# XiSHEN0220/RANSAC-Flow

Hardware: AMD Instinct MI355X
Metric: aligned image-pairs/sec @480×640, 1/2/4/8 MI355X; max-abs flow Δ vs ref (higher is better)
Workload: dtype f32

## Files before the change

### ransac-flow_amd/csrc/conv3x3s.hip

```cpp
#include "common.h"
#include "conv_epilogue.h"
#include "group.h"
#include <stdlib.h>

namespace {

typedef __bf16 bf16x8 __attribute__((ext_vector_type(8)));
typedef __bf16 bf16x2 __attribute__((ext_vector_type(2)));
typedef float f32x2 __attribute__((ext_vector_type(2)));
typedef unsigned u32x4 __attribute__((ext_vector_type(4)));

constexpr int PT_C = 16, PC = PT_C + 2;
template <int WM> struct Geo {
    static constexpr int BM = 64 * WM, WN = 4 / WM, PT_R = 4 * WN, PR = PT_R + 2, PP = PR * PC;
    static constexpr int B_ITEMS = 2 * PP, NBI = (B_ITEMS + 255) / 256;
};

struct C3SArgs {
    const float* in; const u32x4* wS; const float* scale; const float* shift; const float* res; float* out;
    int N, Cin, H, W, Cout, act, Mpad;
    int tilesM, tilesW, tilesS;
};

__device__ __forceinline__ unsigned pack_bf16(float a, float b) {
    const f32x2 v = {a, b};
    const bf16x2 h = __builtin_convertvector(v, bf16x2);
    unsigned u;
    __builtin_memcpy(&u, &h, 4);
    return u;
}
__device__ __forceinline__ void split_pair(float a, float b, unsigned& hi, unsigned& mid, unsigned& lo) {
    hi = pack_bf16(a, b);
    const float ra = a - __uint_as_float(hi << 16), rb = b - __uint_as_float(hi & 0xffff0000u);
    mid = pack_bf16(ra, rb);
    lo = pack_bf16(ra - __uint_as_float(mid << 16), rb - __uint_as_float(mid & 0xffff0000u));
}
__device__ __forceinline__ bf16x8 as_frag(const u32x4& w) {
    bf16x8 f;
    __builtin_memcpy(&f, &w, 16);
    return f;
}

typedef const __attribute__((address_space(1))) void* gptr_t;
typedef __attribute__((address_space(3))) void* lptr_t;

template <int OFF>
__device__ __forceinline__ void lds_rd(u32x4& d, unsigned addr) {
    asm volatile("ds_read_b128 %0, %1 offset:%2" : "=v"(d) : "v"(addr), "n"(OFF));
}
__device__ __forceinline__ void lds_wait8(u32x4& a, u32x4& b, u32x4& c, u32x4& d, u32x4& e, u32x4& f, u32x4& g, u32x4& h) {
    asm volatile("s_waitcnt lgkmcnt(0)" : "+v"(a), "+v"(b), "+v"(c), "+v"(d), "+v"(e), "+v"(f), "+v"(g), "+v"(h));
}
__device__ __forceinline__ void lds_wait4(u32x4& a, u32x4& b, u32x4& c, u32x4& d) {
    asm volatile("s_waitcnt lgkmcnt(0)" : "+v"(a), "+v"(b), "+v"(c), "+v"(d));
}

template <int WM, bool ADMA>
__device__ __forceinline__ void conv3x3_split_body(const C3SArgs& a, const unsigned bx) {
    using G = Geo<WM>;
    constexpr int TM = 2;
    constexpr int BM = G::BM, PT_R = G::PT_R, PP = G::PP, B_ITEMS = G::B_ITEMS, NBI = G::NBI;
    constexpr int A_WORDS = 3 * 2 * BM;
    constexpr int NA = (A_WORDS + 255) / 256;
    __shared__ u32x4 As[2][3][2][BM];
    __shared__ u32x4 Bs[2][3][2][PP];
    __shared__ float s_scale[BM], s_shift[BM];

    const int t = threadIdx.x, lane = t & 63, wave = __builtin_amdgcn_readfirstlane(t >> 6);
    const int wm = WM == 2 ? wave >> 1 : 0, wn = WM == 2 ? wave & 1 : wave;
    const int lrow = lane >> 5, lcol = lane & 31;
    const size_t HW = (size_t)a.H * a.W;
    const int nwg = a.tilesM * a.tilesW * a.tilesS;
    const int nk = a.Cin / 16;
    const int Hs = a.H + 1;

    int m0, row0, col0;
    {
        const int v = (int)bx, q = nwg / 8, r = nwg % 8, xcd = v % 8, j = v / 8;
        int bid = (xcd < r ? xcd * (q + 1) : r * (q + 1) + (xcd - r) * q) + j;
        m0 = (bid % a.tilesM) * BM; bid /= a.tilesM;
        col0 = (bid % a.tilesW) * PT_C;
        row0 = (bid / a.tilesW) * PT_R;
    }
    constexpr int A_ROWS = 256 / BM;
    const u32x4* wsrc = a.wS + (size_t)(t / BM) * a.Mpad + m0 + t % BM;
    auto a_on = [&](int j) { return (j + 1) * 256 <= A_WORDS || t + 256 * j < A_WORDS; };
    const float* bsrc[NBI];
    bool b_ok[NBI], b_on[NBI];
    int b_word[NBI];
#pragma unroll
    for (int u = 0; u < NBI; ++u) {
        const int it = t + 256 * u;
        b_on[u] = it < B_ITEMS;
        const int h = (b_on[u] ? it : 0) / PP, pp = (b_on[u] ? it : 0) % PP;
        const int pr = pp / PC, pc = pp % PC;
        const int sr = row0 - 1 + pr, x = col0 - 1 + pc;
        const int n = sr >= 0 ? sr / Hs : 0, y = sr >= 0 ? sr - n * Hs : 0;
        b_ok[u] = b_on[u] && sr >= 0 && n < a.N && y < a.H && x >= 0 && x < a.W;
        bsrc[u] = b_ok[u] ? a.in + ((size_t)n * a.Cin + 8 * h) * HW + (size_t)y * a.W + x : a.in;
        b_word[u] = h * PP + pp;
    }
    u32x4 ra[NA];
    float rb[8];
    auto load_a = [&](int q) {
#pragma unroll
        for (int j = 0; j < NA; ++j)
            ra[j] = wsrc[((size_t)q * 6 + (a_on(j) ? A_ROWS * j : 0)) * a.Mpad];
    };
    auto store_a = [&](int buf) {
#pragma unroll
        for (int j = 0; j < NA; ++j)
            if (a_on(j)) (&As[buf][0][0][0])[t + 256 * j] = ra[j];
    };
    auto dma_a = [&](int q, int buf) {
#pragma unroll
        for (int j = 0; j < NA; ++j)
            if ((j + 1) * 256 <= A_WORDS || wave < (A_WORDS - 256 * j) / 64)
                __builtin_amdgcn_global_load_lds((gptr_t)(wsrc + ((size_t)q * 6 + A_ROWS * j) * a.Mpad),
                                                 (lptr_t)(&As[buf][0][0][0] + 256 * j + 64 * wave), 16, 0, 0);
    };
    auto load_b = [&](int kb, int u) {
#pragma unroll
        for (int i = 0; i < 8; ++i) rb[i] = bsrc[u][((size_t)kb * 16 + i) * HW];
    };
    auto store_b = [&](int buf, int u) {
        if (!b_on[u]) return;
        u32x4 hi, mid, lo;
#pragma unroll
        for (int i = 0; i < 4; ++i) {
            unsigned h_, m_, l_;
            split_pair(b_ok[u] ? rb[2 * i] : 0.0f, b_ok[u] ? rb[2 * i + 1] : 0.0f, h_, m_, l_);
            hi[i] = h_; mid[i] = m_; lo[i] = l_;
        }
        u32x4* dst = &Bs[buf][0][0][0] + b_word[u];
        dst[0] = hi;
        dst[2 * PP] = mid;
        dst[4 * PP] = lo;
    };
    if (t < BM) {
        const int m = m0 + t;
        s_scale[t] = (a.scale && m < a.Cout) ? a.scale[m] : 1.0f;
        s_shift[t] = (a.shift && m < a.Cout) ? a.shift[m] : 0.0f;
    }
    if (ADMA) dma_a(0, 0);
    else { load_a(0); store_a(0); }
#pragma unroll
    for (int u = 0; u < NBI; ++u) { load_b(0, u); store_b(0, u); }
    if (ADMA) asm volatile("s_waitcnt vmcnt(0)" ::: "memory");
    else load_a(1);
    if (nk > 1) load_b(1, 0);
    __syncthreads();

    f32x16 acc[TM][2], low[TM][2];
#pragma unroll
    for (int i = 0; i < TM; ++i)
#pragma unroll
        for (int j = 0; j < 2; ++j)
#pragma unroll
            for (int r = 0; r < 16; ++r) { acc[i][j][r] = 0.0f; low[i][j][r] = 0.0f; }

    const int a_base = lrow * BM + wm * TM * 32 + lcol;
    int b_base[2];
#pragma unroll
    for (int j = 0; j < 2; ++j) b_base[j] = lrow * PP + (4 * wn + 2 * j + (lcol >> 4)) * PC + (lcol & 15);
    const int nq = 9 * nk;
    const unsigned as_lds = (unsigned)(uintptr_t)(lptr_t)&As[0][0][0][0], bs_lds = (unsigned)(uintptr_t)(lptr_t)&Bs[0][0][0][0];

    for (int kb = 0; kb < nk; ++kb) {
        const u32x4* bimg = &Bs[kb & 1][0][0][0];
#pragma unroll
        for (int tap = 0; tap < 9; ++tap) {
            const int q = kb * 9 + tap;
            const u32x4* aimg = &As[q & 1][0][0][0];
            const int toff = (tap / 3) * PC + tap % 3;
            bf16x8 a0[TM], a1[TM], b0[2], b1[2];
            u32x4 ra0[2], ra1[2], rb0[2], rb1[2];
            unsigned a_addr = 0, b_addr[2] = {0, 0};
            if constexpr (ADMA) {
                static_assert(TM == 2, "hand-written fragment reads: two channel tiles per wavefront");
                a_addr = as_lds + (unsigned)(((q & 1) * A_WORDS + a_base) * 16);
                b_addr[0] = bs_lds + (unsigned)(((kb & 1) * 6 * PP + b_base[0] + toff) * 16);
                b_addr[1] = bs_lds + (unsigned)(((kb & 1) * 6 * PP + b_base[1] + toff) * 16);
                lds_rd<0>(ra0[0], a_addr); lds_rd<512>(ra0[1], a_addr);
                lds_rd<2 * BM * 16>(ra1[0], a_addr); lds_rd<2 * BM * 16 + 512>(ra1[1], a_addr);
                lds_rd<0>(rb0[0], b_addr[0]); lds_rd<0>(rb0[1], b_addr[1]);
                lds_rd<2 * PP * 16>(rb1[0], b_addr[0]); lds_rd<2 * PP * 16>(rb1[1], b_addr[1]);
            } else {
#pragma unroll
                for (int i = 0; i < TM; ++i) {
                    a0[i] = as_frag(aimg[a_base + i * 32]);
                    a1[i] = as_frag(aimg[2 * BM + a_base + i * 32]);
                }
#pragma unroll
                for (int j = 0; j < 2; ++j) {
                    b0[j] = as_frag(bimg[b_base[j] + toff]);
                    b1[j] = as_frag(bimg[2 * PP + b_base[j] + toff]);
                }
            }
            if (!ADMA) {
                if (q + 1 < nq) store_a((q + 1) & 1);
                if (q + 2 < nq) load_a(q + 2);
            }
            int b_next = -1, b_kb = 0;
            if (kb + 1 < nk) {
                if (NBI == 2) {
                    if (tap == 3) { store_b((kb + 1) & 1, 0); b_next = 1; b_kb = kb + 1; }
                    if (tap == 7) store_b((kb + 1) & 1, 1);
                } else {
                    if (tap == 2) { store_b((kb + 1) & 1, 0); b_next = 1; b_kb = kb + 1; }
                    if (tap == 5) { store_b((kb + 1) & 1, 1); b_next = NBI - 1; b_kb = kb + 1; }
                    if (tap == 8) store_b((kb + 1) & 1, NBI - 1);
                }
            }
            if (tap == 8 && kb + 2 < nk) { b_next = 0; b_kb = kb + 2; }
            const bool b_req = b_next >= 0;
            if (ADMA && q + 1 < nq) dma_a(q + 1, (q + 1) & 1);
            if (!ADMA && b_req) { if (b_next == 0) load_b(b_kb, 0); else if (b_next == 1) load_b(b_kb, 1); else load_b(b_kb, NBI - 1); }
            __builtin_amdgcn_sched_barrier(0);
            if constexpr (ADMA) {
                lds_wait8(ra0[0], ra0[1], ra1[0], ra1[1], rb0[0], rb0[1], rb1[0], rb1[1]);
#pragma unroll
                for (int i = 0; i < 2; ++i) { a0[i] = as_frag(ra0[i]); a1[i] = as_frag(ra1[i]); b0[i] = as_frag(rb0[i]); b1[i] = as_frag(rb1[i]); }
            }
#pragma unroll
            for (int i = 0; i < TM; ++i)
#pragma unroll
                for (int j = 0; j < 2; ++j) {
                    low[i][j] = __builtin_amdgcn_mfma_f32_32x32x16_bf16(a1[i], b1[j], low[i][j], 0, 0, 0);
                    low[i][j] = __builtin_amdgcn_mfma_f32_32x32x16_bf16(a1[i], b0[j], low[i][j], 0, 0, 0);
                }
#pragma unroll
            for (int i = 0; i < TM; ++i)
#pragma unroll
                for (int j = 0; j < 2; ++j) low[i][j] = __builtin_amdgcn_mfma_f32_32x32x16_bf16(a0[i], b1[j], low[i][j], 0, 0, 0);
            __builtin_amdgcn_sched_barrier(0);
            if constexpr (ADMA) {
                lds_rd<4 * BM * 16>(ra1[0], a_addr); lds_rd<4 * BM * 16 + 512>(ra1[1], a_addr);
                lds_rd<4 * PP * 16>(rb1[0], b_addr[0]); lds_rd<4 * PP * 16>(rb1[1], b_addr[1]);
            } else {
#pragma unroll
                for (int i = 0; i < TM; ++i) a1[i] = as_frag(aimg[4 * BM + a_base + i * 32]);
#pragma unroll
                for (int j = 0; j < 2; ++j) b1[j] = as_frag(bimg[4 * PP + b_base[j] + toff]);
            }
            if (ADMA && b_req) {
                __builtin_amdgcn_sched_barrier(0);
                if (b_next == 0) load_b(b_kb, 0); else if (b_next == 1) load_b(b_kb, 1); else load_b(b_kb, NBI - 1);
                __builtin_amdgcn_sched_barrier(0);
            }
#pragma unroll
            for (int i = 0; i < TM; ++i)
#pragma unroll
                for (int j = 0; j < 2; ++j) acc[i][j] = __builtin_amdgcn_mfma_f32_32x32x16_bf16(a0[i], b0[j], acc[i][j], 0, 0, 0);
            __builtin_amdgcn_sched_barrier(0);
            if constexpr (ADMA) {
                lds_wait4(ra1[0], ra1[1], rb1[0], rb1[1]);
#pragma unroll
                for (int i = 0; i < 2; ++i) { a1[i] = as_frag(ra1[i]); b1[i] = as_frag(rb1[i]); }
            }
#pragma unroll
            for (int i = 0; i < TM; ++i)
#pragma unroll
                for (int j = 0; j < 2; ++j) {
                    low[i][j] = __builtin_amdgcn_mfma_f32_32x32x16_bf16(a1[i], b0[j], low[i][j], 0, 0, 0);
                    low[i][j] = __builtin_amdgcn_mfma_f32_32x32x16_bf16(a0[i], b1[j], low[i][j], 0, 0, 0);
                }
            __builtin_amdgcn_sched_barrier(0);
            if (ADMA) {
                asm volatile("s_waitcnt vmcnt(0) lgkmcnt(0)" ::: "memory");
                __builtin_amdgcn_s_barrier();
            } else {
                __syncthreads();
            }
        }
    }
#pragma unroll
    for (int i = 0; i < TM; ++i)
#pragma unroll
        for (int j = 0; j < 2; ++j)
#pragma unroll
            for (int r = 0; r < 16; ++r) acc[i][j][r] += low[i][j][r];

    size_t pix_off[2];
    bool pix_ok[2];
#pragma unroll
    for (int j = 0; j < 2; ++j) {
        const int sr = row0 + 4 * wn + 2 * j + (lcol >> 4), x = col0 + (lcol & 15);
        const int n = sr / Hs, y = sr - n * Hs;
        pix_ok[j] = n < a.N && y < a.H && x < a.W;
        pix_off[j] = pix_ok[j] ? (size_t)n * a.Cout * HW + (size_t)y * a.W + x : 0;
    }
    conv_epilogue<TM, 2, false>(acc, s_scale, s_shift, a.res, a.out, a.act, a.Cout, HW, m0, wm, lrow, pix_off, pix_ok, m0 + BM <= a.Cout);
}

template <int TM, bool ADMA>
__global__ __launch_bounds__(256, 2) void conv3x3_split_kernel(C3SArgs a) {
    conv3x3_split_body<TM, ADMA>(a, blockIdx.x);
}

template <int TM, bool ADMA>
__global__ __launch_bounds__(256, 2) void conv3x3_split_group_kernel(RfxGroupArgs<C3SArgs> g) {
    const unsigned y = blockIdx.y;
    if (blockIdx.x >= g.gx[y]) return;
    conv3x3_split_body<TM, ADMA>(g.p[y], blockIdx.x);
}

template <int TM, bool ADMA>
static int c3s_group_launch(const void* blob, const unsigned* gx, int n, hipStream_t st) {
    return rfx_group_launch_impl<C3SArgs>(conv3x3_split_group_kernel<TM, ADMA>, 256, blob, gx, n, st);
}

template <int TM, bool ADMA>
int launch_split3_a(C3SArgs& a, hipStream_t st) {
    a.tilesM = (a.Cout + 64 * TM - 1) / (64 * TM);
    a.tilesW = (a.W + PT_C - 1) / PT_C;
    const long long rows = (long long)a.N * (a.H + 1) - 1;
    a.tilesS = (int)((rows + Geo<TM>::PT_R - 1) / Geo<TM>::PT_R);
    const long long nwg = (long long)a.tilesM * a.tilesW * a.tilesS;
    if (nwg > 0x7fffffffLL) return RFX_E_LIMIT;
    if (rfx_group_recording()) return rfx_group_record(&c3s_group_launch<TM, ADMA>, &a, sizeof(a), (unsigned)nwg);
    hipLaunchKernelGGL((conv3x3_split_kernel<TM, ADMA>), dim3((unsigned)nwg), dim3(256), 0, st, a);
    RFX_LAUNCH_CHECK();
    return RFX_OK;
}

template <int TM>
int launch_split3(C3SArgs& a, hipStream_t st) {
    static const bool adma = !(getenv("RFX_C3S_ADMA") && atoi(getenv("RFX_C3S_ADMA")) == 0);
    return adma ? launch_split3_a<TM, true>(a, st) : launch_split3_a<TM, false>(a, st);
}

constexpr int S2_PR = 2 * 8 + 1, S2_PC = 33, S2_PP = S2_PR * S2_PC;
constexpr int S2_ITEMS = 2 * S2_PP, S2_NBI = (S2_ITEMS + 255) / 256;

struct C3S2Args {
    const float* in; const u32x4* wS; const float* scale; const float* shift; const float* res; float* out;
    int N, Cin, H, W, Ho, Wo, Cout, act, Mpad;
    int tilesM, tilesW, tilesS;
};

__device__ __forceinline__ void conv3x3_split_s2_body(const C3S2Args& a, const unsigned bx) {
    constexpr int TM = 2, BM = 128;
    constexpr int NA = 3;
    __shared__ u32x4 As[2][3][2][BM];
    __shared__ u32x4 Bs[3][2][S2_PP];
    __shared__ float s_scale[BM], s_shift[BM];

    const int t = threadIdx.x, lane = t & 63, wave = __builtin_amdgcn_readfirstlane(t >> 6);
    const int wm = wave >> 1, wn = wave & 1;
    const int lrow = lane >> 5, lcol = lane & 31;
    const size_t HW = (size_t)a.H * a.W, HWo = (size_t)a.Ho * a.Wo;
    const int nwg = a.tilesM * a.tilesW * a.tilesS;
    const int nk = a.Cin / 16;
    const int Hs = a.Ho + 1, Hin = 2 * Hs;

    int m0, row0, col0;
    {
        const int v = (int)bx, q = nwg / 8, r = nwg % 8, xcd = v % 8, j = v / 8;
        int bid = (xcd < r ? xcd * (q + 1) : r * (q + 1) + (xcd - r) * q) + j;
        m0 = (bid % a.tilesM) * BM; bid /= a.tilesM;
        col0 = (bid % a.tilesW) * 16;
        row0 = (bid / a.tilesW) * 8;
    }
    const u32x4* wsrc = a.wS + (size_t)(t / BM) * a.Mpad + m0 + t % BM;
    const float* bsrc[S2_NBI];
    bool b_ok[S2_NBI];
    int b_word[S2_NBI];
#pragma unroll
    for (int u = 0; u < S2_NBI; ++u) {
        const int it = t + 256 * u;
        const bool on = it < S2_ITEMS;
        const int h = (on ? it : 0) / S2_PP, pp = (on ? it : 0) % S2_PP;
        const int pr = pp / S2_PC, pc = pp % S2_PC;
        const int si = 2 * row0 - 1 + pr, x = 2 * col0 - 1 + pc;
        const int n = si >= 0 ? si / Hin : 0, y = si >= 0 ? si - n * Hin : 0;
        b_ok[u] = on && si >= 0 && n < a.N && y < a.H && x >= 0 && x < a.W;
        bsrc[u] = b_ok[u] ? a.in + ((size_t)n * a.Cin + 8 * h) * HW + (size_t)y * a.W + x : a.in;
        b_word[u] = on ? h * S2_PP + pr * S2_PC + (pc & 1) * 17 + (pc >> 1) : -1;
    }
    auto dma_a = [&](int q, int buf) {
#pragma unroll
        for (int j = 0; j < NA; ++j)
            __builtin_amdgcn_global_load_lds((gptr_t)(wsrc + ((size_t)q * 6 + 2 * j) * a.Mpad), (lptr_t)(&As[buf][0][0][0] + 256 * j + 64 * wave),
                                             16, 0, 0);
    };
    auto stage_b = [&](int kb) {
        float rb[4][8];
#pragma unroll
        for (int u = 0; u < 4; ++u)
#pragma unroll
            for (int i = 0; i < 8; ++i) rb[u][i] = bsrc[u][((size_t)kb * 16 + i) * HW];
        auto put = [&](const float (&v)[8], int u) {
            if (b_word[u] < 0) return;
            u32x4 hi, mid, lo;
#pragma unroll
            for (int i = 0; i < 4; ++i) {
                unsigned h_, m_, l_;
                split_pair(b_ok[u] ? v[2 * i] : 0.0f, b_ok[u] ? v[2 * i + 1] : 0.0f, h_, m_, l_);
                hi[i] = h_; mid[i] = m_; lo[i] = l_;
            }
            u32x4* dst = &Bs[0][0][0] + b_word[u];
            dst[0] = hi;
            dst[2 * S2_PP] = mid;
            dst[4 * S2_PP] = lo;
        };
#pragma unroll
        for (int u = 0; u < 4; ++u) put(rb[u], u);
        float r4[8];
#pragma unroll
        for (int i = 0; i < 8; ++i) r4[i] = bsrc[4][((size_t)kb * 16 + i) * HW];
        put(r4, 4);
    };
    if (t < BM) {
        const int m = m0 + t;
        s_scale[t] = (a.scale && m < a.Cout) ? a.scale[m] : 1.0f;
        s_shift[t] = (a.shift && m < a.Cout) ? a.shift[m] : 0.0f;
    }
    dma_a(0, 0);

    f32x16 acc[TM][2], low[TM][2];
#pragma unroll
    for (int i = 0; i < TM; ++i)
#pragma unroll
        for (int j = 0; j < 2; ++j)
#pragma unroll
            for (int r = 0; r < 16; ++r) { acc[i][j][r] = 0.0f; low[i][j][r] = 0.0f; }

    const int a_base = lrow * BM + wm * TM * 32 + lcol;
    int b_base[2];
#pragma unroll
    for (int j = 0; j < 2; ++j) b_base[j] = lrow * S2_PP + 2 * (4 * wn + 2 * j + (lcol >> 4)) * S2_PC + (lcol & 15);
    const int nq = 9 * nk;
    const u32x4* bimg = &Bs[0][0][0];

    for (int kb = 0; kb < nk; ++kb) {
        stage_b(kb);
        asm volatile("s_waitcnt vmcnt(0)" ::: "memory");
        __syncthreads();
#pragma unroll
        for (int tap = 0; tap < 9; ++tap) {
            const int q = kb * 9 + tap;
            const u32x4* aimg = &As[q & 1][0][0][0];
            const int toff = (tap / 3) * S2_PC + (tap % 3 & 1) * 17 + (tap % 3 >> 1);
            bf16x8 a0[TM], a1[TM], b0[2], b1[2];
#pragma unroll
            for (int i = 0; i < TM; ++i) {
                a0[i] = as_frag(aimg[a_base + i * 32]);
                a1[i] = as_frag(aimg[2 * BM + a_base + i * 32]);
            }
#pragma unroll
            for (int j = 0; j < 2; ++j) {
                b0[j] = as_frag(bimg[b_base[j] + toff]);
                b1[j] = as_frag(bimg[2 * S2_PP + b_base[j] + toff]);
            }
            if (q + 1 < nq) dma_a(q + 1, (q + 1) & 1);
            __builtin_amdgcn_sched_barrier(0);
#pragma unroll
            for (int i = 0; i < TM; ++i)
#pragma unroll
                for (int j = 0; j < 2; ++j) {
                    low[i][j] = __builtin_amdgcn_mfma_f32_32x32x16_bf16(a1[i], b1[j], low[i][j], 0, 0, 0);
                    low[i][j] = __builtin_amdgcn_mfma_f32_32x32x16_bf16(a1[i], b0[j], low[i][j], 0, 0, 0);
                }
#pragma unroll
            for (int i = 0; i < TM; ++i)
#pragma unroll
                for (int j = 0; j < 2; ++j) low[i][j] = __builtin_amdgcn_mfma_f32_32x32x16_bf16(a0[i], b1[j], low[i][j], 0, 0, 0);
            __builtin_amdgcn_sched_barrier(0);
#pragma unroll
            for (int i = 0; i < TM; ++i) a1[i] = as_frag(aimg[4 * BM + a_base + i * 32]);
#pragma unroll
            for (int j = 0; j < 2; ++j) b1[j] = as_frag(bimg[4 * S2_PP + b_base[j] + toff]);
#pragma unroll
            for (int i = 0; i < TM; ++i)
#pragma unroll
                for (int j = 0; j < 2; ++j) acc[i][j] = __builtin_amdgcn_mfma_f32_32x32x16_bf16(a0[i], b0[j], acc[i][j], 0, 0, 0);
            __builtin_amdgcn_sched_barrier(0);
#pragma unroll
            for (int i = 0; i < TM; ++i)
#pragma unroll
                for (int j = 0; j < 2; ++j) {
                    low[i][j] = __builtin_amdgcn_mfma_f32_32x32x16_bf16(a1[i], b0[j], low[i][j], 0, 0, 0);
                    low[i][j] = __builtin_amdgcn_mfma_f32_32x32x16_bf16(a0[i], b1[j], low[i][j], 0, 0, 0);
                }
            __builtin_amdgcn_sched_barrier(0);
            asm volatile("s_waitcnt vmcnt(0)" ::: "memory");
            __syncthreads();
        }
    }
#pragma unroll
    for (int i = 0; i < TM; ++i)
#pragma unroll
        for (int j = 0; j < 2; ++j)
#pragma unroll
            for (int r = 0; r < 16; ++r) acc[i][j][r] += low[i][j][r];

    size_t pix_off[2];
    bool pix_ok[2];
#pragma unroll
    for (int j = 0; j < 2; ++j) {
        const int sr = row0 + 4 * wn + 2 * j + (lcol >> 4), x = col0 + (lcol & 15);
        const int n = sr / Hs, y = sr - n * Hs;
        pix_ok[j] = n < a.N && y < a.Ho && x < a.Wo;
        pix_off[j] = pix_ok[j] ? (size_t)n * a.Cout * HWo + (size_t)y * a.Wo + x : 0;
    }
    conv_epilogue<TM, 2, false>(acc, s_scale, s_shift, a.res, a.out, a.act, a.Cout, HWo, m0, wm, lrow, pix_off, pix_ok, m0 + BM <= a.Cout);
}

__global__ __launch_bounds__(256, 2) void conv3x3_split_s2_kernel(C3S2Args a) {
    conv3x3_split_s2_body(a, blockIdx.x);
}

__global__ __launch_bounds__(256, 2) void conv3x3_split_s2_group_kernel(RfxGroupArgs<C3S2Args> g) {
    const unsigned y = blockIdx.y;
    if (blockIdx.x >= g.gx[y]) return;
    conv3x3_split_s2_body(g.p[y], blockIdx.x);
}

static int c3s2_group_launch(const void* blob, const unsigned* gx, int n, hipStream_t st) {
    return rfx_group_launch_impl<C3S2Args>(conv3x3_split_s2_group_kernel, 256, blob, gx, n, st);
}

}

extern "C" int rfx_conv3x3_split_f32(const float* in, const void* wS3, const float* scale, const float* shift, const float* residual,
                                     float* out, int N, int Cin, int H, int W, int Cout, int act, void* stream) {
    if (!in || !wS3 || !out || N <= 0 || Cin <= 0 || H <= 0 || W <= 0 || Cout <= 0) return RFX_E_ARG;
    if (Cin % 16 != 0) return RFX_E_ARG;
    if (act != RFX_ACT_NONE && act != RFX_ACT_RELU && act != RFX_ACT_SIGMOID) return RFX_E_ARG;
    if ((long long)N * (H + 1) > 0x7fffffffLL) return RFX_E_LIMIT;
    C3SArgs a;
    a.in = in; a.wS = reinterpret_cast<const u32x4*>(wS3); a.scale = scale; a.shift = shift; a.res = residual; a.out = out;
    a.N = N; a.Cin = Cin; a.H = H; a.W = W; a.Cout = Cout; a.act = act; a.Mpad = (Cout + 127) / 128 * 128;
    return Cout > 64 ? launch_split3<2>(a, rfx_stream(stream)) : launch_split3<1>(a, rfx_stream(stream));
}

extern "C" int rfx_conv3x3_split_s2_f32(const float* in, const void* wS3, const float* scale, const float* shift, const float* residual,
                                        float* out, int N, int Cin, int H, int W, int Cout, int act, void* stream) {
    if (!in || !wS3 || !out || N <= 0 || Cin <= 0 || H <= 0 || W <= 0 || Cout <= 0) return RFX_E_ARG;
    if (Cin % 16 != 0) return RFX_E_ARG;
    if (act != RFX_ACT_NONE && act != RFX_ACT_RELU && act != RFX_ACT_SIGMOID) return RFX_E_ARG;
    C3S2Args a;
    a.in = in; a.wS = reinterpret_cast<const u32x4*>(wS3); a.scale = scale; a.shift = shift; a.res = residual; a.out = out;
    a.N = N; a.Cin = Cin; a.H = H; a.W = W; a.Ho = (H - 1) / 2 + 1; a.Wo = (W - 1) / 2 + 1; a.Cout = Cout; a.act = act;
    a.Mpad = (Cout + 127) / 128 * 128;
    if ((long long)N * (a.Ho + 1) * 2 > 0x7fffffffLL) return RFX_E_LIMIT;
    a.tilesM = (Cout + 127) / 128;
    a.tilesW = (a.Wo + 15) / 16;
    a.tilesS = (int)(((long long)N * (a.Ho + 1) - 1 + 7) / 8);
    const long long nwg = (long long)a.tilesM * a.tilesW * a.tilesS;
    if (nwg > 0x7fffffffLL) return RFX_E_LIMIT;
    hipStream_t st = rfx_stream(stream);
    if (rfx_group_recording()) return rfx_group_record(&c3s2_group_launch, &a, sizeof(a), (unsigned)nwg);
    hipLaunchKernelGGL(conv3x3_split_s2_kernel, dim3((unsigned)nwg), dim3(256), 0, st, a);
    RFX_LAUNCH_CHECK();
    return RFX_OK;
}
```

Before: 163.9.

## Prefetch next-tap B fragments during MFMAs and swizzle lane-row mapping in conv3x3

Software-pipelines the B-operand LDS reads so the fragments for the next tap are issued between MFMA groups of the current tap and consumed without a fresh wait. It also adds a lane-to-row swizzle for the B tile, intended to reduce LDS bank conflicts, and converts the stride-2 kernel to hand-issued ds_read_b128 with a raw s_barrier. The aim is to hide LDS read latency behind MFMA work, at the cost of extra live VGPRs, which could pressure occupancy at launch_bounds(256,2).

```diff
diff --git a/ransac-flow_amd/csrc/conv3x3s.hip b/ransac-flow_amd/csrc/conv3x3s.hip
--- a/ransac-flow_amd/csrc/conv3x3s.hip
+++ b/ransac-flow_amd/csrc/conv3x3s.hip
@@ -54,6 +54,12 @@
 __device__ __forceinline__ void lds_wait4(u32x4& a, u32x4& b, u32x4& c, u32x4& d) {
     asm volatile("s_waitcnt lgkmcnt(0)" : "+v"(a), "+v"(b), "+v"(c), "+v"(d));
 }
+
+__device__ __forceinline__ int c3s_lane_row(int lcol) { return (lcol >> 4) ^ (((lcol >> 2) ^ (lcol >> 3)) & 1); }
+
+#ifndef RFX_C3S_BPREFETCH
+#define RFX_C3S_BPREFETCH 1
+#endif
 
 template <int WM, bool ADMA>
 __device__ __forceinline__ void conv3x3_split_body(const C3SArgs& a, const unsigned bx) {
@@ -162,9 +168,20 @@
     const int a_base = lrow * BM + wm * TM * 32 + lcol;
     int b_base[2];
 #pragma unroll
-    for (int j = 0; j < 2; ++j) b_base[j] = lrow * PP + (4 * wn + 2 * j + (lcol >> 4)) * PC + (lcol & 15);
+    for (int j = 0; j < 2; ++j) b_base[j] = lrow * PP + (4 * wn + 2 * j + c3s_lane_row(lcol)) * PC + (lcol & 15);
     const int nq = 9 * nk;
     const unsigned as_lds = (unsigned)(uintptr_t)(lptr_t)&As[0][0][0][0], bs_lds = (unsigned)(uintptr_t)(lptr_t)&Bs[0][0][0][0];
+    constexpr bool BPF = ADMA && RFX_C3S_BPREFETCH;
+    constexpr bool BPF_WRAP = BPF && NBI == 2;
+    u32x4 nb0[2] = {}, nb1[2] = {};
+    if constexpr (BPF_WRAP) {
+#pragma unroll
+        for (int j = 0; j < 2; ++j) {
+            const unsigned nb_addr = bs_lds + (unsigned)(b_base[j] * 16);
+            lds_rd<0>(nb0[j], nb_addr); lds_rd<2 * PP * 16>(nb1[j], nb_addr);
+        }
+        lds_wait4(nb0[0], nb0[1], nb1[0], nb1[1]);
+    }
 
     for (int kb = 0; kb < nk; ++kb) {
         const u32x4* bimg = &Bs[kb & 1][0][0][0];
@@ -176,6 +193,7 @@
             bf16x8 a0[TM], a1[TM], b0[2], b1[2];
             u32x4 ra0[2], ra1[2], rb0[2], rb1[2];
             unsigned a_addr = 0, b_addr[2] = {0, 0};
+            const bool have_pf = BPF && (tap > 0 || BPF_WRAP), do_pf = BPF && (tap < 8 || BPF_WRAP);
             if constexpr (ADMA) {
                 static_assert(TM == 2, "hand-written fragment reads: two channel tiles per wavefront");
                 a_addr = as_lds + (unsigned)(((q & 1) * A_WORDS + a_base) * 16);
@@ -183,8 +201,10 @@
                 b_addr[1] = bs_lds + (unsigned)(((kb & 1) * 6 * PP + b_base[1] + toff) * 16);
                 lds_rd<0>(ra0[0], a_addr); lds_rd<512>(ra0[1], a_addr);
                 lds_rd<2 * BM * 16>(ra1[0], a_addr); lds_rd<2 * BM * 16 + 512>(ra1[1], a_addr);
-                lds_rd<0>(rb0[0], b_addr[0]); lds_rd<0>(rb0[1], b_addr[1]);
-                lds_rd<2 * PP * 16>(rb1[0], b_addr[0]); lds_rd<2 * PP * 16>(rb1[1], b_addr[1]);
+                if (!have_pf) {
+                    lds_rd<0>(rb0[0], b_addr[0]); lds_rd<0>(rb0[1], b_addr[1]);
+                    lds_rd<2 * PP * 16>(rb1[0], b_addr[0]); lds_rd<2 * PP * 16>(rb1[1], b_addr[1]);
+                }
             } else {
 #pragma unroll
                 for (int i = 0; i < TM; ++i) {
@@ -218,17 +238,40 @@
             if (!ADMA && b_req) { if (b_next == 0) load_b(b_kb, 0); else if (b_next == 1) load_b(b_kb, 1); else load_b(b_kb, NBI - 1); }
             __builtin_amdgcn_sched_barrier(0);
             if constexpr (ADMA) {
-                lds_wait8(ra0[0], ra0[1], ra1[0], ra1[1], rb0[0], rb0[1], rb1[0], rb1[1]);
+                if (have_pf) {
+                    lds_wait4(ra0[0], ra0[1], ra1[0], ra1[1]);
+#pragma unroll
+                    for (int j = 0; j < 2; ++j) { rb0[j] = nb0[j]; rb1[j] = nb1[j]; }
+                } else {
+                    lds_wait8(ra0[0], ra0[1], ra1[0], ra1[1], rb0[0], rb0[1], rb1[0], rb1[1]);
+                }
 #pragma unroll
                 for (int i = 0; i < 2; ++i) { a0[i] = as_frag(ra0[i]); a1[i] = as_frag(ra1[i]); b0[i] = as_frag(rb0[i]); b1[i] = as_frag(rb1[i]); }
             }
-#pragma unroll
-            for (int i = 0; i < TM; ++i)
+            unsigned nb_addr[2] = {0, 0};
+            if (do_pf) {
+                const int toff_n = ((tap + 1) / 3) * PC + (tap + 1) % 3;
+#pragma unroll
+                for (int j = 0; j < 2; ++j)
+                    nb_addr[j] = tap < 8 ? b_addr[j] + (unsigned)((toff_n - toff) * 16)
+                                         : bs_lds + (unsigned)((((kb + 1) & 1) * 6 * PP + b_base[j]) * 16);
+            }
+#pragma unroll
+            for (int i = 0; i < TM; ++i) {
 #pragma unroll
                 for (int j = 0; j < 2; ++j) {
                     low[i][j] = __builtin_amdgcn_mfma_f32_32x32x16_bf16(a1[i], b1[j], low[i][j], 0, 0, 0);
                     low[i][j] = __builtin_amdgcn_mfma_f32_32x32x16_bf16(a1[i], b0[j], low[i][j], 0, 0, 0);
                 }
+                if constexpr (ADMA) {
+                    if (do_pf) {
+                        __builtin_amdgcn_sched_barrier(0);
+                        if (i == 0) { lds_rd<0>(nb0[0], nb_addr[0]); lds_rd<0>(nb0[1], nb_addr[1]); }
+                        else { lds_rd<2 * PP * 16>(nb1[0], nb_addr[0]); lds_rd<2 * PP * 16>(nb1[1], nb_addr[1]); }
+                        __builtin_amdgcn_sched_barrier(0);
+                    }
+                }
+            }
 #pragma unroll
             for (int i = 0; i < TM; ++i)
 #pragma unroll
@@ -254,7 +297,8 @@
                 for (int j = 0; j < 2; ++j) acc[i][j] = __builtin_amdgcn_mfma_f32_32x32x16_bf16(a0[i], b0[j], acc[i][j], 0, 0, 0);
             __builtin_amdgcn_sched_barrier(0);
             if constexpr (ADMA) {
-                lds_wait4(ra1[0], ra1[1], rb1[0], rb1[1]);
+                if (do_pf) lds_wait8(ra1[0], ra1[1], rb1[0], rb1[1], nb0[0], nb0[1], nb1[0], nb1[1]);
+                else lds_wait4(ra1[0], ra1[1], rb1[0], rb1[1]);
 #pragma unroll
                 for (int i = 0; i < 2; ++i) { a1[i] = as_frag(ra1[i]); b1[i] = as_frag(rb1[i]); }
             }
@@ -285,7 +329,7 @@
     bool pix_ok[2];
 #pragma unroll
     for (int j = 0; j < 2; ++j) {
-        const int sr = row0 + 4 * wn + 2 * j + (lcol >> 4), x = col0 + (lcol & 15);
+        const int sr = row0 + 4 * wn + 2 * j + c3s_lane_row(lcol), x = col0 + (lcol & 15);
         const int n = sr / Hs, y = sr - n * Hs;
         pix_ok[j] = n < a.N && y < a.H && x < a.W;
         pix_off[j] = pix_ok[j] ? (size_t)n * a.Cout * HW + (size_t)y * a.W + x : 0;
@@ -385,11 +429,13 @@
                                              16, 0, 0);
     };
     auto stage_b = [&](int kb) {
+        size_t hw = HW;
+        asm volatile("" : "+s"(hw));
         float rb[4][8];
 #pragma unroll
         for (int u = 0; u < 4; ++u)
 #pragma unroll
-            for (int i = 0; i < 8; ++i) rb[u][i] = bsrc[u][((size_t)kb * 16 + i) * HW];
+            for (int i = 0; i < 8; ++i) rb[u][i] = bsrc[u][((size_t)kb * 16 + i) * hw];
         auto put = [&](const float (&v)[8], int u) {
             if (b_word[u] < 0) return;
             u32x4 hi, mid, lo;
@@ -408,7 +454,7 @@
         for (int u = 0; u < 4; ++u) put(rb[u], u);
         float r4[8];
 #pragma unroll
-        for (int i = 0; i < 8; ++i) r4[i] = bsrc[4][((size_t)kb * 16 + i) * HW];
+        for (int i = 0; i < 8; ++i) r4[i] = bsrc[4][((size_t)kb * 16 + i) * hw];
         put(r4, 4);
     };
     if (t < BM) {
@@ -429,9 +475,11 @@
     const int a_base = lrow * BM + wm * TM * 32 + lcol;
     int b_base[2];
 #pragma unroll
-    for (int j = 0; j < 2; ++j) b_base[j] = lrow * S2_PP + 2 * (4 * wn + 2 * j + (lcol >> 4)) * S2_PC + (lcol & 15);
+    for (int j = 0; j < 2; ++j) b_base[j] = lrow * S2_PP + 2 * (4 * wn + 2 * j + c3s_lane_row(lcol)) * S2_PC + (lcol & 15);
     const int nq = 9 * nk;
-    const u32x4* bimg = &Bs[0][0][0];
+    const unsigned as_lds = (unsigned)(uintptr_t)(lptr_t)&As[0][0][0][0], bs_lds = (unsigned)(uintptr_t)(lptr_t)&Bs[0][0][0];
+    constexpr bool BPF = RFX_C3S_BPREFETCH;
+    u32x4 nb0[2] = {}, nb1[2] = {};
 
     for (int kb = 0; kb < nk; ++kb) {
         stage_b(kb);
@@ -440,42 +488,62 @@
 #pragma unroll
         for (int tap = 0; tap < 9; ++tap) {
             const int q = kb * 9 + tap;
-            const u32x4* aimg = &As[q & 1][0][0][0];
             const int toff = (tap / 3) * S2_PC + (tap % 3 & 1) * 17 + (tap % 3 >> 1);
             bf16x8 a0[TM], a1[TM], b0[2], b1[2];
+            u32x4 ra0[2], ra1[2], rb0[2], rb1[2];
+            const unsigned a_addr = as_lds + (unsigned)(((q & 1) * 6 * BM + a_base) * 16);
+            const unsigned b_addr[2] = {bs_lds + (unsigned)((b_base[0] + toff) * 16), bs_lds + (unsigned)((b_base[1] + toff) * 16)};
+            lds_rd<0>(ra0[0], a_addr); lds_rd<512>(ra0[1], a_addr);
+            lds_rd<2 * BM * 16>(ra1[0], a_addr); lds_rd<2 * BM * 16 + 512>(ra1[1], a_addr);
+            const bool have_pf = BPF && tap > 0, do_pf = BPF && tap < 8;
+            if (!have_pf) {
+                lds_rd<0>(rb0[0], b_addr[0]); lds_rd<0>(rb0[1], b_addr[1]);
+                lds_rd<2 * S2_PP * 16>(rb1[0], b_addr[0]); lds_rd<2 * S2_PP * 16>(rb1[1], b_addr[1]);
+            }
+            if (q + 1 < nq) dma_a(q + 1, (q + 1) & 1);
+            __builtin_amdgcn_sched_barrier(0);
+            if (have_pf) {
+                lds_wait4(ra0[0], ra0[1], ra1[0], ra1[1]);
+#pragma unroll
+                for (int j = 0; j < 2; ++j) { rb0[j] = nb0[j]; rb1[j] = nb1[j]; }
+            } else {
+                lds_wait8(ra0[0], ra0[1], ra1[0], ra1[1], rb0[0], rb0[1], rb1[0], rb1[1]);
+            }
+#pragma unroll
+            for (int i = 0; i < 2; ++i) { a0[i] = as_frag(ra0[i]); a1[i] = as_frag(ra1[i]); b0[i] = as_frag(rb0[i]); b1[i] = as_frag(rb1[i]); }
+            const int tapn = tap < 8 ? tap + 1 : tap;
+            const int toff_n = (tapn / 3) * S2_PC + (tapn % 3 & 1) * 17 + (tapn % 3 >> 1);
+            const unsigned nb_addr[2] = {b_addr[0] + (unsigned)((toff_n - toff) * 16), b_addr[1] + (unsigned)((toff_n - toff) * 16)};
 #pragma unroll
             for (int i = 0; i < TM; ++i) {
-                a0[i] = as_frag(aimg[a_base + i * 32]);
-                a1[i] = as_frag(aimg[2 * BM + a_base + i * 32]);
-            }
-#pragma unroll
-            for (int j = 0; j < 2; ++j) {
-                b0[j] = as_frag(bimg[b_base[j] + toff]);
-                b1[j] = as_frag(bimg[2 * S2_PP + b_base[j] + toff]);
-            }
-            if (q + 1 < nq) dma_a(q + 1, (q + 1) & 1);
-            __builtin_amdgcn_sched_barrier(0);
-#pragma unroll
-            for (int i = 0; i < TM; ++i)
 #pragma unroll
                 for (int j = 0; j < 2; ++j) {
                     low[i][j] = __builtin_amdgcn_mfma_f32_32x32x16_bf16(a1[i], b1[j], low[i][j], 0, 0, 0);
                     low[i][j] = __builtin_amdgcn_mfma_f32_32x32x16_bf16(a1[i], b0[j], low[i][j], 0, 0, 0);
                 }
+                if (do_pf) {
+                    __builtin_amdgcn_sched_barrier(0);
+                    if (i == 0) { lds_rd<0>(nb0[0], nb_addr[0]); lds_rd<0>(nb0[1], nb_addr[1]); }
+                    else { lds_rd<2 * S2_PP * 16>(nb1[0], nb_addr[0]); lds_rd<2 * S2_PP * 16>(nb1[1], nb_addr[1]); }
+                    __builtin_amdgcn_sched_barrier(0);
+                }
+            }
 #pragma unroll
             for (int i = 0; i < TM; ++i)
 #pragma unroll
                 for (int j = 0; j < 2; ++j) low[i][j] = __builtin_amdgcn_mfma_f32_32x32x16_bf16(a0[i], b1[j], low[i][j], 0, 0, 0);
             __builtin_amdgcn_sched_barrier(0);
-#pragma unroll
-            for (int i = 0; i < TM; ++i) a1[i] = as_frag(aimg[4 * BM + a_base + i * 32]);
-#pragma unroll
-            for (int j = 0; j < 2; ++j) b1[j] = as_frag(bimg[4 * S2_PP + b_base[j] + toff]);
+            lds_rd<4 * BM * 16>(ra1[0], a_addr); lds_rd<4 * BM * 16 + 512>(ra1[1], a_addr);
+            lds_rd<4 * S2_PP * 16>(rb1[0], b_addr[0]); lds_rd<4 * S2_PP * 16>(rb1[1], b_addr[1]);
 #pragma unroll
             for (int i = 0; i < TM; ++i)
 #pragma unroll
                 for (int j = 0; j < 2; ++j) acc[i][j] = __builtin_amdgcn_mfma_f32_32x32x16_bf16(a0[i], b0[j], acc[i][j], 0, 0, 0);
             __builtin_amdgcn_sched_barrier(0);
+            if (do_pf) lds_wait8(ra1[0], ra1[1], rb1[0], rb1[1], nb0[0], nb0[1], nb1[0], nb1[1]);
+            else lds_wait4(ra1[0], ra1[1], rb1[0], rb1[1]);
+#pragma unroll
+            for (int i = 0; i < 2; ++i) { a1[i] = as_frag(ra1[i]); b1[i] = as_frag(rb1[i]); }
 #pragma unroll
             for (int i = 0; i < TM; ++i)
 #pragma unroll
@@ -484,8 +552,8 @@
                     low[i][j] = __builtin_amdgcn_mfma_f32_32x32x16_bf16(a0[i], b1[j], low[i][j], 0, 0, 0);
                 }
             __builtin_amdgcn_sched_barrier(0);
-            asm volatile("s_waitcnt vmcnt(0)" ::: "memory");
-            __syncthreads();
+            asm volatile("s_waitcnt vmcnt(0) lgkmcnt(0)" ::: "memory");
+            __builtin_amdgcn_s_barrier();
         }
     }
 #pragma unroll
@@ -499,7 +567,7 @@
     bool pix_ok[2];
 #pragma unroll
     for (int j = 0; j < 2; ++j) {
-        const int sr = row0 + 4 * wn + 2 * j + (lcol >> 4), x = col0 + (lcol & 15);
+        const int sr = row0 + 4 * wn + 2 * j + c3s_lane_row(lcol), x = col0 + (lcol & 15);
         const int n = sr / Hs, y = sr - n * Hs;
         pix_ok[j] = n < a.N && y < a.Ho && x < a.Wo;
         pix_off[j] = pix_ok[j] ? (size_t)n * a.Cout * HWo + (size_t)y * a.Wo + x : 0;
```

New measurement: 165.3 (median of 6 runs). No clear change (+0.9%).
